# vovach777/llcomp

Measured on AMD Instinct MI355X. Metric: encode+decode MPix/s on 4K RGB8, bit-exact, higher is better.
Workload: dtype int32

## Files before the change

### llcomp_amd/csrc/dec_rows_asm.hpp

```cpp
#pragma once
#include <cstdint>

namespace llcomp_mi {

#define LD_E0L "v32"
#define LD_E0H "v33"
#define LD_E0 "v[32:33]"
#define LD_E5L "v34"
#define LD_E5H "v35"
#define LD_E5 "v[34:35]"
#define LD_E6L "v36"
#define LD_E6H "v37"
#define LD_E6 "v[36:37]"
#define LD_E7L "v38"
#define LD_E7H "v39"
#define LD_E7 "v[38:39]"
#define LD_E1L "v40"
#define LD_E1H "v41"
#define LD_E1 "v[40:41]"
#define LD_E2L "v42"
#define LD_E2H "v43"
#define LD_E2 "v[42:43]"
#define LD_E3L "v44"
#define LD_E3H "v45"
#define LD_E3 "v[44:45]"
#define LD_E4L "v48"
#define LD_E4H "v49"
#define LD_E4 "v[48:49]"
#define LD_PROD "v50"
#define LD_R1 "v51"
#define LD_DIFF "v52"
#define LD_OFF "v52"
#define LD_EX "v32"
#define LD_W "v33"
#define LD_RUN "v40"
#define LD_NX "v41"
#define LD_T "v42"
#define LD_SX "s[56:57]"
#define LD_SA "s[58:59]"
#define LD_SW "s[60:61]"
#define LD_SP "s[62:63]"
#define LD_S5 "s[64:65]"
#define LD_SU "s[66:67]"
#define LD_SD "s[68:69]"
#define LD_S1L "s[68:69]"
#define LD_SM "s[70:71]"
#define LD_S1 "s70"
#define LD_S2 "s71"

#define LD_SPLIT(EL)                                                                                                       \
    "v_mul_u32_u24_sdwa " LD_PROD ", " EL ", %[range] dst_sel:DWORD dst_unused:UNUSED_PAD src0_sel:BYTE_1 src1_sel:DWORD\n\t" \
    "v_lshrrev_b32_e32 " LD_R1 ", 8, " LD_PROD "\n\t"                                                                      \
    "v_sub_u32_e32 %[range], %[range], " LD_R1 "\n\t"
#define LD_SPLIT_IN(EL)                                                                                                       \
    "v_mul_u32_u24_sdwa " LD_PROD ", " EL ", %[range_in] dst_sel:DWORD dst_unused:UNUSED_PAD src0_sel:BYTE_1 src1_sel:DWORD\n\t" \
    "v_lshrrev_b32_e32 " LD_R1 ", 8, " LD_PROD "\n\t"                                                                      \
    "v_sub_u32_e32 %[range], %[range_in], " LD_R1 "\n\t"
#define LD_REFILL(N)                                         \
    "v_cmp_gt_u32_e32 vcc, %[c100], %[range]\n\t"            \
    "s_and_saveexec_b64 " LD_SW ", vcc\n\t"                  \
    "s_cbranch_execz .Lrf" N "_%=\n\t"                       \
    "v_lshlrev_b32_e32 %[range], 8, %[range]\n\t"            \
    "v_perm_b32 %[low], %[low], %[w32], %[sel]\n\t"          \
    "v_lshrrev_b32_e32 %[w32], 8, %[w32]\n"                   \
    ".Lrf" N "_%=:\n\t"                                      \
    "s_mov_b64 exec, " LD_SW "\n\t"
#define LD_REFILL_R1(N)                                           \
    "v_cmp_gt_u32_e32 vcc, %[c100], " LD_R1 "\n\t"                \
    "s_and_saveexec_b64 " LD_SW ", vcc\n\t"                       \
    "s_cbranch_execz .Lrf" N "_%=\n\t"                            \
    "v_and_b32_e32 %[range], 0xffffff00, " LD_PROD "\n\t"         \
    "v_perm_b32 %[low], %[low], %[w32], %[sel]\n\t"               \
    "v_lshrrev_b32_e32 %[w32], 8, %[w32]\n"                        \
    ".Lrf" N "_%=:\n\t"                                           \
    "s_mov_b64 exec, " LD_SW "\n\t"
#define LD_UNARY(EL, EH, OFS, N, SAVE)                                      \
    LD_SPLIT(EL)                                                            \
    "v_sub_co_u32_e32 %[low], vcc, %[low], %[range]\n\t"                    \
    "ds_write_b16_d16_hi %[bank], " EL " offset:" OFS "\n\t"                \
    "s_andn2_b64 exec, exec, vcc\n\t"                                       \
    SAVE                                                                    \
    "s_cbranch_execz .Lx_done_%=\n\t"                                       \
    "ds_write_b16_d16_hi %[bank], " EH " offset:" OFS "\n\t"                \
    "v_add_u32_e32 " LD_EX ", 1, " LD_EX "\n\t"                                     \
    "v_mov_b32_e32 %[range], " LD_R1 "\n\t"                                 \
    LD_REFILL_R1(N)
#define LD_FETCH_REST                                         \
    "v_lshrrev_b32_e32 " LD_E1L ", 16, %[w0]\n\t"             \
    "v_and_b32_e32 " LD_E2L ", 0xffff, %[w1]\n\t"             \
    "v_lshrrev_b32_e32 " LD_E3L ", 16, %[w1]\n\t"             \
    "v_and_b32_e32 " LD_E4L ", 0xffff, %[w2]\n\t"             \
    "ds_read_b64 " LD_E1 ", " LD_E1L "\n\t"                   \
    "ds_read_b64 " LD_E2 ", " LD_E2L "\n\t"                   \
    "ds_read_b64 " LD_E3 ", " LD_E3L "\n\t"                   \
    "ds_read_b64 " LD_E4 ", " LD_E4L "\n\t"                   \
    "v_lshrrev_b32_e32 " LD_E5L ", 16, %[w2]\n\t"             \
    "v_and_b32_e32 " LD_E6L ", 0xffff, %[w3]\n\t"             \
    "v_lshrrev_b32_e32 " LD_E7L ", 16, %[w3]\n\t"             \
    "ds_read_b64 " LD_E5 ", " LD_E5L "\n\t"                   \
    "ds_read_b64 " LD_E6 ", " LD_E6L "\n\t"                   \
    "ds_read_b64 " LD_E7 ", " LD_E7L "\n\t"

__device__ __forceinline__ void dec_rows_sample_asm(uint32_t low_in, uint32_t range_in, unsigned long long win_in, uint32_t& low,
                                                    uint32_t& range, unsigned long long& win, uint32_t w0, uint32_t w1, uint32_t w2,
                                                    uint32_t w3, uint32_t bank, uint32_t& hot, uint32_t& value, uint32_t& w32) {
    asm volatile(
        "s_mov_b64 " LD_SX ", exec\n\t"
        "v_and_b32_e32 %[w32], 0xffffff, %[winl_in]\n\t"
        "v_or_b32_e32 %[w32], 0x1000000, %[w32]\n\t"
        "v_and_b32_e32 " LD_OFF ", 0xffff, %[w0]\n\t"
        "ds_read_b64 " LD_E0 ", " LD_OFF "\n\t"
        "v_mov_b32_e32 %[value], 0\n\t"
        "s_cmp_lg_u32 %[hot], 0\n\t"
        "s_cbranch_scc0 .Lcold_%=\n\t"
        LD_FETCH_REST
        "s_waitcnt lgkmcnt(7)\n\t"
        "s_branch .Lzero_%=\n"
        ".Lcold_%=:\n\t"
        "s_waitcnt lgkmcnt(0)\n"
        ".Lzero_%=:\n\t"
        LD_SPLIT_IN(LD_E0L)
        "v_sub_co_u32_e32 %[low], vcc, %[low_in], %[range]\n\t"
        "ds_write_b16_d16_hi %[bank], " LD_E0L "\n\t"
        "s_and_b64 " LD_SA ", exec, vcc\n\t"
        "v_cndmask_b32_e32 %[low], %[low], %[low_in], vcc\n\t"
        "s_andn2_b64 exec, exec, vcc\n\t"
        "s_cbranch_execz .Lz1_%=\n\t"
        "v_mov_b32_e32 %[range], " LD_R1 "\n\t"
        "ds_write_b16_d16_hi %[bank], " LD_E0H "\n"
        ".Lz1_%=:\n\t"
        "s_mov_b64 exec, " LD_SX "\n\t"
        LD_REFILL("0")
        "s_and_b64 exec, " LD_SA ", " LD_SA "\n\t"
        "s_cbranch_execz .Ldone_%=\n\t"
        "s_cmp_lg_u32 %[hot], 0\n\t"
        "s_cbranch_scc1 .Lhave_%=\n\t"
        LD_FETCH_REST
        ".Lhave_%=:\n\t"
        "v_mov_b32_e32 " LD_EX ", 0\n\t"
        "v_mov_b32_e32 " LD_W ", 1\n\t"
        "s_waitcnt lgkmcnt(0)\n\t"
        "s_mov_b64 " LD_SM ", 0\n\t"
        LD_UNARY(LD_E1L, LD_E1H, "2", "1", "s_mov_b64 " LD_S1L ", exec\n\t")
        LD_UNARY(LD_E2L, LD_E2H, "256", "2", "s_mov_b64 " LD_SM ", exec\n\t")
        LD_UNARY(LD_E3L, LD_E3H, "258", "3", "")
        "s_mov_b64 " LD_SU ", exec\n\t"
        ".p2align 6\n"
        ".Lu_%=:\n\t"
        "s_waitcnt lgkmcnt(0)\n\t"
        LD_SPLIT(LD_E4L)
        "v_sub_co_u32_e32 %[low], vcc, %[low], %[range]\n\t"
        "s_andn2_b64 exec, exec, vcc\n\t"
        "s_cbranch_execz .Lu_done_%=\n\t"
        "v_lshrrev_b32_e32 " LD_OFF ", 16, " LD_E4H "\n\t"
        "ds_read_b64 " LD_E4 ", " LD_OFF "\n\t"
        "v_add_u32_e32 " LD_EX ", 1, " LD_EX "\n\t"
        "v_mov_b32_e32 %[range], " LD_R1 "\n\t"
        LD_REFILL_R1("4")
        "s_branch .Lu_%=\n"
        ".Lu_done_%=:\n\t"
        "s_mov_b64 exec, " LD_SU "\n\t"
        "ds_write_b16_d16_hi %[bank], " LD_E4L " offset:512\n"
        ".Lx_done_%=:\n\t"
        "s_mov_b64 exec, " LD_SA "\n\t"
        "v_add_u32_e32 %[low], %[low], %[range]\n\t"
        LD_REFILL("5")
        "v_cmp_lt_u32_e32 vcc, 31, " LD_EX "\n\t"
        "s_cbranch_vccz .Lexok_%=\n\t"
        "s_and_saveexec_b64 " LD_SP ", vcc\n\t"
        "v_mov_b32_e32 %[w32], 0\n\t"
        "s_andn2_b64 exec, " LD_SP ", exec\n\t"
        "s_cbranch_execz .Ldone_%=\n"
        ".Lexok_%=:\n\t"
        "s_mov_b64 " LD_S5 ", exec\n\t"
        "s_and_b64 exec, exec, " LD_S1L "\n\t"
        "s_cbranch_execz .Lvalue_%=\n\t"
        "s_mov_b64 " LD_SU ", exec\n\t"
        LD_SPLIT(LD_E5L)
        "v_sub_co_u32_e32 " LD_DIFF ", vcc, %[low], %[range]\n\t"
        "ds_write_b16_d16_hi %[bank], " LD_E5L " offset:514\n\t"
        "s_andn2_b64 " LD_SP ", exec, vcc\n\t"
        "v_addc_co_u32_e32 " LD_W ", vcc, " LD_W ", " LD_W ", vcc\n\t"
        "v_mov_b32_e32 " LD_RUN ", 0\n\t"
        "s_and_b64 exec, " LD_SP ", " LD_SP "\n\t"
        "s_cbranch_execz .Lp5_%=\n\t"
        "v_mov_b32_e32 %[low], " LD_DIFF "\n\t"
        "v_mov_b32_e32 %[range], " LD_R1 "\n\t"
        "ds_write_b16_d16_hi %[bank], " LD_E5H " offset:514\n"
        ".Lp5_%=:\n\t"
        "s_mov_b64 exec, " LD_SU "\n\t"
        LD_REFILL("6")
        "v_add_u32_e32 " LD_T ", -1, " LD_EX "\n\t"
        "s_and_b64 exec, exec, " LD_SM "\n\t"
        "s_cbranch_execz .Lm_skip_%=\n\t"
        "s_mov_b64 " LD_SP ", exec\n\t"
        "v_add_u32_e32 " LD_NX ", -2, " LD_EX "\n\t"
        "v_lshrrev_b32_e32 " LD_RUN ", " LD_NX ", %[sentv]\n\t"
        ".p2align 6\n"
        ".Lm_%=:\n\t"
        "s_waitcnt lgkmcnt(0)\n\t"
        LD_SPLIT(LD_E6L)
        "v_sub_co_u32_e32 " LD_DIFF ", vcc, %[low], %[range]\n\t"
        "s_nop 1\n\t"
        "v_cndmask_b32_e32 %[range], " LD_R1 ", %[range], vcc\n\t"
        "v_cndmask_b32_e32 %[low], " LD_DIFF ", %[low], vcc\n\t"
        "v_cndmask_b32_e32 " LD_NX ", " LD_E6H ", " LD_E6L ", vcc\n\t"
        "v_addc_co_u32_e32 " LD_RUN ", vcc, " LD_RUN ", " LD_RUN ", vcc\n\t"
        "s_mov_b64 " LD_SD ", vcc\n\t"
        "v_lshrrev_b32_e32 " LD_OFF ", 16, " LD_NX "\n\t"
        "ds_read_b64 " LD_E6 ", " LD_OFF "\n\t"
        "v_cmp_gt_u32_e32 vcc, %[c100], %[range]\n\t"
        "s_and_saveexec_b64 " LD_SW ", vcc\n\t"
        "s_cbranch_execz .Lmr_%=\n\t"
        "v_lshlrev_b32_e32 %[range], 8, %[range]\n\t"
        "v_perm_b32 %[low], %[low], %[w32], %[sel]\n\t"
        "v_lshrrev_b32_e32 %[w32], 8, %[w32]\n"
        ".Lmr_%=:\n\t"
        "s_andn2_b64 exec, " LD_SW ", " LD_SD "\n\t"
        "s_cbranch_execnz .Lm_%=\n\t"
        "s_mov_b64 exec, " LD_SP "\n\t"
        "ds_write_b16_d16_hi %[bank], " LD_NX " offset:768\n"
        ".Lm_skip_%=:\n\t"
        "s_mov_b64 exec, " LD_SU "\n\t"
        "v_lshlrev_b32_e32 " LD_W ", " LD_T ", " LD_W "\n\t"
        "v_or_b32_e32 " LD_W ", " LD_W ", " LD_RUN "\n"
        ".Lvalue_%=:\n\t"
        "s_mov_b64 exec, " LD_S5 "\n\t"
        "v_lshlrev_b32_e64 " LD_T ", " LD_EX ", 1\n\t"
        "v_add_u32_e32 " LD_T ", -1, " LD_T "\n\t"
        "v_xor_b32_e32 %[value], " LD_W ", " LD_T "\n\t"
        LD_SPLIT(LD_E7L)
        "v_sub_co_u32_e32 " LD_DIFF ", vcc, %[low], %[range]\n\t"
        "ds_write_b16_d16_hi %[bank], " LD_E7L " offset:770\n\t"
        "s_andn2_b64 exec, exec, vcc\n\t"
        "s_cbranch_execz .Lp7_%=\n\t"
        "v_mov_b32_e32 %[low], " LD_DIFF "\n\t"
        "v_mov_b32_e32 %[range], " LD_R1 "\n\t"
        "ds_write_b16_d16_hi %[bank], " LD_E7H " offset:770\n\t"
        "v_sub_u32_e32 %[value], 0, %[value]\n"
        ".Lp7_%=:\n\t"
        "s_mov_b64 exec, " LD_S5 "\n\t"
        LD_REFILL("7")
        ".Ldone_%=:\n\t"
        "s_mov_b64 exec, " LD_SX "\n\t"
        "v_ffbh_u32_e32 " LD_DIFF ", %[w32]\n\t"
        "v_add_u32_e32 " LD_DIFF ", -7, " LD_DIFF "\n\t"
        "v_lshrrev_b64 %[win], " LD_DIFF ", %[win_in]\n\t"
        "s_bcnt1_i32_b64 " LD_S1 ", " LD_SA "\n\t"
        "s_bcnt1_i32_b64 " LD_S2 ", " LD_SX "\n\t"
        "s_lshl_b32 " LD_S1 ", " LD_S1 ", 1\n\t"
        "s_cmp_ge_u32 " LD_S1 ", " LD_S2 "\n\t"
        "s_cselect_b32 %[hot], 1, 0\n\t"
        "s_mov_b64 exec, " LD_SX "\n\t"
        : [low] "=&v"(low), [range] "=&v"(range), [win] "=&v"(win), [hot] "+s"(hot), [value] "=&v"(value), [w32] "=&v"(w32)
        : [low_in] "v"(low_in), [range_in] "v"(range_in), [win_in] "v"(win_in), [winl_in] "v"(uint32_t(win_in)), [w0] "v"(w0), [w1] "v"(w1), [w2] "v"(w2), [w3] "v"(w3), [bank] "v"(bank), [c100] "s"(0x100u), [sel] "s"(0x06050400u),
          [sentv] "v"(0x80000000u)
        : "vcc", "scc", "memory", "v32", "v33", "v34", "v35", "v36", "v37", "v38", "v39", "v40", "v41", "v42", "v43", "v44", "v45",
          "v48", "v49", "v50", "v51", "v52", "s56", "s57", "s58", "s59", "s60", "s61", "s62", "s63", "s64", "s65", "s66",
          "s67", "s68", "s69", "s70", "s71");
}

}
```

### llcomp_amd/csrc/slice_kernels.hip

```cpp
#include <algorithm>
#include <type_traits>

#include "device_common.hpp"
#include "kernels.hpp"

#ifndef LLMI_ASM_ENC
#define LLMI_ASM_ENC 1
#endif
#if LLMI_ASM_ENC
#include "enc_rows_asm.hpp"
#endif
#ifndef LLMI_ASM_DEC
#define LLMI_ASM_DEC 1
#endif
#if LLMI_ASM_DEC
#include "dec_rows_asm.hpp"
#endif

namespace llcomp_mi {

namespace {

#ifdef LLMI_CLOCK_PROBE
constexpr uint32_t kProbeSlots = 1u << 15;
// ... 869 lines not shown
    bool ok = true;
    if (dec_once<1, CHECKED, INLDS>(d, bank, E)) {
        ex = 1;
        if (dec_once<2, CHECKED, INLDS>(d, bank, E)) {
            ex = 2;
            if (dec_once<3, CHECKED, INLDS>(d, bank, E)) {
                entry_t cur = E.e4;
                int n = 0;
                for (;;) {
                    if (CHECKED && d.win <= 1) dec_append_drained(d);
                    const uint32_t r1 = __umul24(d.range, prob_of(cur)) >> 8;
                    d.range -= r1;
                    ++n;
                    asm volatile("" : "+v"(n));
                    uint32_t diff;
                    if (__builtin_usub_overflow(d.low, d.range, &diff)) break;
                    d.low = diff;
                    d.range = r1;
                    if (CHECKED && n > 29) break;
                    cur = entry_at(tab, uint32_t(cur >> 32));
                    dec_refill(d);
                }
                dec_refill(d);
                ex = 2 + n;
                if (ex > 31) ok = false;
                const uint32_t nx = uint32_t(cur);
                dec_put_state<4, INLDS>(bank, nx);
            }
        }
    }
    if (!ok) return false;
    uint32_t w = 1;
    const uint32_t ones = (1u << ex) - 1;
    if (ex > 0) {
        w += w + uint32_t(!dec_once<5, CHECKED, INLDS>(d, bank, E));
        if (ex > 1) {
            entry_t cur = E.e6;
            uint32_t nx;
            uint32_t limit = ones + 1;
            asm volatile("" : "+v"(limit));
            do {
                nx = dec_step_acc<CHECKED>(d, prob_of(cur), cur, w);
                cur = entry_at(tab, nx);
            } while (w < limit);
            dec_put_state<6, INLDS>(bank, nx);
        }
    }
    uint32_t v = w ^ ones;
    if (dec_once<7, CHECKED, INLDS>(d, bank, E)) v = 0u - v;
    out = v;
    return true;
}

template <bool INLDS>
__device__ __forceinline__ bool dec_sample(RangeDec& d, Bank& bank, const entry_t* tab, uint32_t& hot, bool replay_always,
                                           uint32_t& v) {
#if LLMI_ASM_DEC
    if constexpr (INLDS) {
        uint32_t low, range, left;
        unsigned long long win;
        dec_rows_sample_asm(d.low, d.range, d.win, low, range, win, bank.w[0], bank.w[1], bank.w[2], bank.w[3], lds_address(bank.lds), hot, v,
                            left);
        if (__builtin_expect(left == 0 || replay_always, 0)) {
            ++d.replays;
            reinterpret_cast<uint32_t*>(bank.lds)[0] = bank.w[0];
            reinterpret_cast<uint32_t*>(bank.lds)[64] = bank.w[1];
            reinterpret_cast<uint32_t*>(bank.lds)[128] = bank.w[2];
            reinterpret_cast<uint32_t*>(bank.lds)[192] = bank.w[3];
            asm("v_mov_b32_e32 %0, %3\n\tv_mov_b32_e32 %1, %4\n\tv_mov_b64_e32 %2, %5"
                : "+v"(low), "+v"(range), "+v"(win)
                : "v"(d.low), "v"(d.range), "v"(d.win));
            d.low = low;
            d.range = range;
            d.win = win;
            return dec_residual<false, true, true>(d, bank, tab, v);
        }
        d.low = low;
        d.range = range;
        d.win = win;
        return true;
    } else
#endif
    {
        const uint32_t s_low = d.low, s_range = d.range, s_b0 = bank.w[0], s_b1 = bank.w[1], s_b2 = bank.w[2], s_b3 = bank.w[3];
        const unsigned long long s_win = d.win;
        bool ok = hot ? dec_residual<true, false, INLDS>(d, bank, tab, v) : dec_residual<false, false, INLDS>(d, bank, tab, v);
        hot = 2 * __popcll(__ballot(v != 0)) >= __popcll(__ballot(true));
        if (__builtin_expect(!ok || d.win == 0 || replay_always, 0)) {
            ++d.replays;
            d.low = s_low; d.range = s_range; d.win = s_win;
            bank.w[0] = s_b0; bank.w[1] = s_b1;
            if constexpr (INLDS) {
                bank.w[2] = s_b2; bank.w[3] = s_b3;
                reinterpret_cast<uint32_t*>(bank.lds)[0] = s_b0;
                reinterpret_cast<uint32_t*>(bank.lds)[64] = s_b1;
                reinterpret_cast<uint32_t*>(bank.lds)[128] = s_b2;
                reinterpret_cast<uint32_t*>(bank.lds)[192] = s_b3;
            }
            ok = dec_residual<false, true, INLDS>(d, bank, tab, v);
        }
        return ok;
    }
}

constexpr uint32_t bank_cache_lds_bytes(int log2_entries) { return log2_entries ? (64u * 9u) << log2_entries : 0u; }
template <int NCH, bool ROWS, bool LDSTAB = false, int CACHE = 0, bool SMALL = false>
__global__ __launch_bounds__(64, ROWS && NCH == 1 ? 8 : 1) void k_decode_slices(const Geometry g, const uint32_t lpw_and_flags,
                                                      const uint8_t* __restrict__ units,
                                                      const uint32_t* __restrict__ slice_len,
                                                      uint64_t* __restrict__ states, int16_t* __restrict__ rec,
                                                      uint32_t* status, const uint64_t gpat,
                                                      unsigned long long* __restrict__ counters) {
    __shared__ entry_t tab[128];
    __shared__ uint32_t rowbank[ROWS ? kWideBankWords : 1];
    __shared__ int8_t quant_lut[ROWS ? 1 : 512];
    if constexpr (!ROWS) {
        for (uint32_t i = threadIdx.x; i < 256; i += blockDim.x) {
            quant_lut[i] = int8_t(quant11(int(i) - 128));
            quant_lut[256 + i] = int8_t(quant5(int(i) - 128));
        }
    }
    static_assert(CACHE == 0 || (!ROWS && !LDSTAB && NCH != 0), "the bank cache belongs to the 2-D kernels with tables in HBM");
    static_assert(!SMALL || ROWS, "the model is a template flag of the 1-row-slice kernels only");
    static_assert(CACHE == 0 || ((kContexts - 1) >> CACHE) < 0xFF, "bank cache: a context's tag would alias the empty marker");
    __shared__ uint32_t wave_sums[CACHE != 0 ? 2 : 1];
    clear_lds_states<LDSTAB>();
    if constexpr (CACHE != 0) {
        uint32_t* tg = reinterpret_cast<uint32_t*>(dyn_lds + (512u << CACHE));
        for (uint32_t i = threadIdx.x; i < (16u << CACHE); i += blockDim.x) tg[i] = 0xFFFFFFFFu;
        if (threadIdx.x < 2) wave_sums[threadIdx.x] = 0;
    }
    load_table(tab);
    const uint32_t lpw = lpw_and_flags & 0xFF;
    const bool replay_always = (lpw_and_flags >> 8) & 1;
    [[maybe_unused]] const bool small_model = (g.flags & kGeoSmallModel) != 0;
    const uint32_t id = blockIdx.x * lpw + threadIdx.x;
    if (threadIdx.x >= lpw || id >= g.n_slices) return;
    const SliceRect r = slice_rect(g, id);
    RangeDec d;
    const uint32_t len = min(slice_len[id], g.slice_cap - 16);
    const uint32_t grp = __builtin_amdgcn_readfirstlane(id >> g.lane_shift);
    const uint32_t lane_in_group = id & ((1u << g.lane_shift) - 1);
    dec_open(d, reinterpret_cast<const uint32_t*>(units) + ((size_t(grp) * (g.slice_cap >> 2)) << g.lane_shift), lane_in_group,
             g.lane_shift, len);

    int16_t* p0 = rec + lane_order_index(g, id, 0);
    const ptrdiff_t GW = ptrdiff_t(1) << g.lane_shift;
    int16_t* const gbase = rec + ((size_t(grp) * g.slice_samples) << g.lane_shift);
    uint32_t hot = 0;
    LLMI_PROBE_START();

    if constexpr (ROWS) {
        for (uint32_t k = 0; k < 12; ++k) rowbank[k * 64 + threadIdx.x] = lds_address(tab) * 0x00010001u;
        int l[NCH], L[NCH];
#pragma unroll
        for (int k = 0; k < NCH; ++k) l[k] = L[k] = 128;
        int held_val = 0;
        uint32_t store_ofs = lane_in_group * 2, step_ofs = 2u << g.lane_shift;
        asm volatile("" : "+v"(step_ofs));
        uint8_t* const bank0 = reinterpret_cast<uint8_t*>(rowbank) + threadIdx.x * 4;
        bool bad = false;
        auto pixel = [&](auto model, auto start) {
            constexpr int MODEL = decltype(model)::value;
            constexpr bool START = decltype(start)::value;
#pragma unroll
            for (int k = 0; k < NCH; ++k) {
                if (window_low(d)) dec_append(d);
                if (!(START && k == 0)) {
                    asm volatile("global_store_short %0, %1, %2" : : "v"(store_ofs), "v"(held_val), "s"(gbase) : "memory");
                    store_ofs += step_ofs;
                }
                const int lv = l[k];
                uint32_t sg = 0, bofs = 0;
                if constexpr (MODEL != kModelSmall) {
                    const int dq = L[k] - lv;
                    sg = uint32_t(dq >> 31);
                    asm volatile("" : "+v"(sg));
                    const uint32_t aq = (uint32_t(dq) ^ sg) - sg;
                    uint32_t o1 = ((aq + 0x7FFFFFFFu) >> 21) & 0x400u, o2 = ((aq + 0x7FFFFFFCu) >> 21) & 0x400u;
                    asm volatile("" : "+v"(o1), "+v"(o2));
                    bofs = o1 + o2;
                }
                uint32_t* bp = reinterpret_cast<uint32_t*>(bank0 + bofs);
                Bank bank{{bp[0], bp[64], bp[128], bp[192]}, reinterpret_cast<uint8_t*>(bp)};
                uint32_t v = 0;
                if (!dec_sample<true>(d, bank, tab, hot, replay_always, v)) bad = true;
                if constexpr (MODEL != kModelSmall) v = (v ^ sg) - sg;
                const int val = int(int16_t(uint32_t(lv) + v));
                held_val = val;
                L[k] = START ? val : lv;
                l[k] = val;
            }
        };
        const uint32_t sw0 = __builtin_amdgcn_readfirstlane(r.sw);
        const uint32_t n_bulk = __builtin_amdgcn_ballot_w64(r.sw != sw0) == 0 ? sw0 : 0;
        uint32_t x = 1;
        pixel(no_model, std::true_type{});
        constexpr std::integral_constant<int, SMALL ? kModelSmall : kModelLarge> model{};
        if constexpr (NCH == 1) {
            for (; x + 1 < n_bulk; x += 2) {
                pixel(model, std::false_type{});
                pixel(model, std::false_type{});
            }
        } else {
            for (; x < n_bulk; ++x) pixel(model, std::false_type{});
        }
        for (; x < r.sw; ++x) pixel(model, std::false_type{});
        if (bad) atomicOr(status, kStBadExponent);
        asm volatile("global_store_short %0, %1, %2" : : "v"(store_ofs), "v"(held_val), "s"(gbase) : "memory");
        publish_count(counters, kCtrDecReplays, d.replays);
    } else {
        uint64_t* banks;
        uint32_t bsh;
        if constexpr (LDSTAB) {
            banks = reinterpret_cast<uint64_t*>(dyn_lds);
            bsh = 0;
        } else {
            banks = states + ((size_t(id >> g.lane_shift) * kContexts) << g.lane_shift) + (id & ((1u << g.lane_shift) - 1));
            bsh = g.lane_shift;
        }
        if constexpr (NCH == 0) {
            const uint32_t nch = g.nch;
            const ptrdiff_t px_step = ptrdiff_t(nch) * GW, up = ptrdiff_t(r.sw) * px_step;
            for (uint32_t y = 0; y < r.sh; ++y) {
                for (uint32_t x = 0; x < r.sw; ++x) {
                    for (uint32_t k = 0; k < nch; ++k) {
                        int16_t* q = p0 + ptrdiff_t(y) * up + ptrdiff_t(x) * px_step + ptrdiff_t(k) * GW;
                        if (window_low(d)) dec_append(d);
                        const Hood n = apply_borders(x > 0 ? q[-px_step] : 0, x > 1 ? q[-2 * px_step] : 0, y > 0 ? q[-up] : 0,
                                                     (y > 0 && x > 0) ? q[-up - px_step] : 0, (y > 0 && x + 1 < r.sw) ? q[-up + px_step] : 0,
                                                     y > 1 ? q[-2 * up] : 0, x, y, r.sw);
                        int ctx = context_hash(n, small_model);
                        const bool neg = ctx < 0;
                        if (neg) ctx = -ctx;
                        const uint64_t b64 = bank_fresh<LDSTAB>(banks[size_t(ctx) << bsh], gpat);
                        Bank bank{{uint32_t(b64), uint32_t(b64 >> 32)}, nullptr};
                        uint32_t v;
                        if (!dec_sample<false>(d, bank, tab, hot, replay_always, v)) {
                            atomicOr(status, kStBadExponent);
                            return;
                        }
                                banks[size_t(ctx) << bsh] = bank_tagged<LDSTAB>(uint64_t(bank.w[0]) | (uint64_t(bank.w[1]) << 32), gpat);
                        if (neg) v = 0u - v;
                        *q = int16_t(uint32_t(predict(n)) + v);
                    }
                }
            }
            publish_count(counters, kCtrDecReplays, d.replays);
        } else {
        const ptrdiff_t up = ptrdiff_t(r.sw) * NCH * GW;
        uint32_t held_ctx = ~0u;
        uint64_t held_bank = 0;
        [[maybe_unused]] uint64_t wb_bank = 0;
        [[maybe_unused]] uint64_t* wb_ptr = nullptr;
        [[maybe_unused]] bool use_cache = CACHE != 0;
        [[maybe_unused]] uint32_t my_miss = 0, my_lookups = 0, my_wb = 0, miss_mark = 0, look_mark = 0;
        LLMI_PARTS_DECL();
        LLMI_PARTS_START();
        for (uint32_t y = 0; y < r.sh; ++y) {
            if constexpr (CACHE != 0) {
// ... 273 lines not shown
```

Before: 30460.

## Pack decoder low and byte window into a 64-bit register pair with alternating sets

Rewrites the row-decoder inline assembly so the range-coder low value and the pending refill bytes sit in one 64-bit register pair. A refill then becomes a single 64-bit shift in place of a perm plus a shift. The unary-run loop is unrolled by two, with range and R1 swapping roles so the register move per step disappears. Consecutive samples alternate between two fixed register pairs (v0:1 / v2:3), which lets the compiler overlap them and avoid copies. The cost is hard-pinned physical registers and more complex asm that must stay bit-exact.

```diff
diff --git a/llcomp_amd/csrc/dec_rows_asm.hpp b/llcomp_amd/csrc/dec_rows_asm.hpp
--- a/llcomp_amd/csrc/dec_rows_asm.hpp
+++ b/llcomp_amd/csrc/dec_rows_asm.hpp
@@ -41,6 +41,7 @@
 #define LD_SW "s[60:61]"
 #define LD_SP "s[62:63]"
 #define LD_S5 "s[64:65]"
+#define LD_SB "s[64:65]"
 #define LD_SU "s[66:67]"
 #define LD_SD "s[68:69]"
 #define LD_S1L "s[68:69]"
@@ -56,35 +57,37 @@
     "v_mul_u32_u24_sdwa " LD_PROD ", " EL ", %[range_in] dst_sel:DWORD dst_unused:UNUSED_PAD src0_sel:BYTE_1 src1_sel:DWORD\n\t" \
     "v_lshrrev_b32_e32 " LD_R1 ", 8, " LD_PROD "\n\t"                                                                      \
     "v_sub_u32_e32 %[range], %[range_in], " LD_R1 "\n\t"
+#define LD_SPLIT_TO(EL, RD, WR)                                                                                       \
+    "v_mul_u32_u24_sdwa " LD_PROD ", " EL ", " RD " dst_sel:DWORD dst_unused:UNUSED_PAD src0_sel:BYTE_1 src1_sel:DWORD\n\t" \
+    "v_lshrrev_b32_e32 " WR ", 8, " LD_PROD "\n\t"                                                                     \
+    "v_sub_u32_e32 " RD ", " RD ", " WR "\n\t"
+#define LD_TAKE "v_lshlrev_b64 " LD_PAIR ", 8, " LD_PAIR "\n"
 #define LD_REFILL(N)                                         \
     "v_cmp_gt_u32_e32 vcc, %[c100], %[range]\n\t"            \
     "s_and_saveexec_b64 " LD_SW ", vcc\n\t"                  \
     "s_cbranch_execz .Lrf" N "_%=\n\t"                       \
     "v_lshlrev_b32_e32 %[range], 8, %[range]\n\t"            \
-    "v_perm_b32 %[low], %[low], %[w32], %[sel]\n\t"          \
-    "v_lshrrev_b32_e32 %[w32], 8, %[w32]\n"                   \
+    LD_TAKE                                                  \
     ".Lrf" N "_%=:\n\t"                                      \
     "s_mov_b64 exec, " LD_SW "\n\t"
-#define LD_REFILL_R1(N)                                           \
-    "v_cmp_gt_u32_e32 vcc, %[c100], " LD_R1 "\n\t"                \
+#define LD_REFILL_R1(WR, N)                                       \
+    "v_cmp_gt_u32_e32 vcc, %[c100], " WR "\n\t"                   \
     "s_and_saveexec_b64 " LD_SW ", vcc\n\t"                       \
     "s_cbranch_execz .Lrf" N "_%=\n\t"                            \
-    "v_and_b32_e32 %[range], 0xffffff00, " LD_PROD "\n\t"         \
-    "v_perm_b32 %[low], %[low], %[w32], %[sel]\n\t"               \
-    "v_lshrrev_b32_e32 %[w32], 8, %[w32]\n"                        \
+    "v_and_b32_e32 " WR ", 0xffffff00, " LD_PROD "\n\t"           \
+    LD_TAKE                                                       \
     ".Lrf" N "_%=:\n\t"                                           \
     "s_mov_b64 exec, " LD_SW "\n\t"
-#define LD_UNARY(EL, EH, OFS, N, SAVE)                                      \
-    LD_SPLIT(EL)                                                            \
-    "v_sub_co_u32_e32 %[low], vcc, %[low], %[range]\n\t"                    \
+#define LD_UNARY(EL, EH, OFS, N, SAVE, RD, WR)                              \
+    LD_SPLIT_TO(EL, RD, WR)                                                 \
+    "v_sub_co_u32_e32 " LD_LOW ", vcc, " LD_LOW ", " RD "\n\t"              \
     "ds_write_b16_d16_hi %[bank], " EL " offset:" OFS "\n\t"                \
     "s_andn2_b64 exec, exec, vcc\n\t"                                       \
     SAVE                                                                    \
     "s_cbranch_execz .Lx_done_%=\n\t"                                       \
     "ds_write_b16_d16_hi %[bank], " EH " offset:" OFS "\n\t"                \
-    "v_add_u32_e32 " LD_EX ", 1, " LD_EX "\n\t"                                     \
-    "v_mov_b32_e32 %[range], " LD_R1 "\n\t"                                 \
-    LD_REFILL_R1(N)
+    "v_add_u32_e32 " LD_EX ", 1, " LD_EX "\n\t"                             \
+    LD_REFILL_R1(WR, N)
 #define LD_FETCH_REST                                         \
     "v_lshrrev_b32_e32 " LD_E1L ", 16, %[w0]\n\t"             \
     "v_and_b32_e32 " LD_E2L ", 0xffff, %[w1]\n\t"             \
@@ -101,163 +104,233 @@
     "ds_read_b64 " LD_E6 ", " LD_E6L "\n\t"                   \
     "ds_read_b64 " LD_E7 ", " LD_E7L "\n\t"
 
-__device__ __forceinline__ void dec_rows_sample_asm(uint32_t low_in, uint32_t range_in, unsigned long long win_in, uint32_t& low,
-                                                    uint32_t& range, unsigned long long& win, uint32_t w0, uint32_t w1, uint32_t w2,
-                                                    uint32_t w3, uint32_t bank, uint32_t& hot, uint32_t& value, uint32_t& w32) {
-    asm volatile(
-        "s_mov_b64 " LD_SX ", exec\n\t"
-        "v_and_b32_e32 %[w32], 0xffffff, %[winl_in]\n\t"
-        "v_or_b32_e32 %[w32], 0x1000000, %[w32]\n\t"
-        "v_and_b32_e32 " LD_OFF ", 0xffff, %[w0]\n\t"
-        "ds_read_b64 " LD_E0 ", " LD_OFF "\n\t"
-        "v_mov_b32_e32 %[value], 0\n\t"
-        "s_cmp_lg_u32 %[hot], 0\n\t"
-        "s_cbranch_scc0 .Lcold_%=\n\t"
-        LD_FETCH_REST
-        "s_waitcnt lgkmcnt(7)\n\t"
-        "s_branch .Lzero_%=\n"
-        ".Lcold_%=:\n\t"
-        "s_waitcnt lgkmcnt(0)\n"
-        ".Lzero_%=:\n\t"
-        LD_SPLIT_IN(LD_E0L)
-        "v_sub_co_u32_e32 %[low], vcc, %[low_in], %[range]\n\t"
-        "ds_write_b16_d16_hi %[bank], " LD_E0L "\n\t"
-        "s_and_b64 " LD_SA ", exec, vcc\n\t"
-        "v_cndmask_b32_e32 %[low], %[low], %[low_in], vcc\n\t"
-        "s_andn2_b64 exec, exec, vcc\n\t"
-        "s_cbranch_execz .Lz1_%=\n\t"
-        "v_mov_b32_e32 %[range], " LD_R1 "\n\t"
-        "ds_write_b16_d16_hi %[bank], " LD_E0H "\n"
-        ".Lz1_%=:\n\t"
+#define LD_HEAD_COPY "v_perm_b32 " LD_CPY ", %[winl_in], %[winl_in], %[sel]\n\t"
+#define LD_SEL 0x0001020Du
+#define LD_TAIL_BITS "v_ffbl_b32_e32 " LD_DIFF ", " LD_CPY "\n\t"
+#define LD_URUN                                                      \
+    ".Lu_%=:\n\t"                                                    \
+    "s_waitcnt lgkmcnt(0)\n\t"                                       \
+    LD_SPLIT_TO(LD_E4L, LD_R1, "%[range]")                           \
+    "v_sub_co_u32_e32 " LD_LOW ", vcc, " LD_LOW ", " LD_R1 "\n\t"    \
+    "s_and_b64 " LD_SP ", exec, vcc\n\t"                             \
+    "s_andn2_b64 exec, exec, vcc\n\t"                                \
+    "s_or_b64 " LD_SB ", " LD_SB ", " LD_SP "\n\t"                   \
+    "s_cbranch_execz .Lu_done_%=\n\t"                                \
+    "v_lshrrev_b32_e32 " LD_OFF ", 16, " LD_E4H "\n\t"               \
+    "ds_read_b64 " LD_E4 ", " LD_OFF "\n\t"                          \
+    "v_add_u32_e32 " LD_EX ", 1, " LD_EX "\n\t"                      \
+    LD_REFILL_R1("%[range]", "4")                                    \
+    "s_waitcnt lgkmcnt(0)\n\t"                                       \
+    LD_SPLIT_TO(LD_E4L, "%[range]", LD_R1)                           \
+    "v_sub_co_u32_e32 " LD_LOW ", vcc, " LD_LOW ", %[range]\n\t"     \
+    "s_andn2_b64 exec, exec, vcc\n\t"                                \
+    "s_cbranch_execz .Lu_done_%=\n\t"                                \
+    "v_lshrrev_b32_e32 " LD_OFF ", 16, " LD_E4H "\n\t"               \
+    "ds_read_b64 " LD_E4 ", " LD_OFF "\n\t"                          \
+    "v_add_u32_e32 " LD_EX ", 1, " LD_EX "\n\t"                      \
+    LD_REFILL_R1(LD_R1, "4b")                                        \
+    "s_branch .Lu_%=\n"
+#define LD_UNARY_INIT "s_mov_b64 " LD_SB ", 0\n\t"
+#define LD_SAVE2 "s_mov_b64 " LD_SM ", exec\n\ts_andn2_b64 " LD_SB ", " LD_S1L ", exec\n\t"
+#define LD_COLLECT                           \
+    "s_mov_b64 exec, " LD_SB "\n\t"          \
+    "v_mov_b32_e32 %[range], " LD_R1 "\n\t"
+
+#define LD_TEXT                                                                                                                    \
+        "s_mov_b64 " LD_SX ", exec\n\t"                                                                                            \
+        LD_HEAD_COPY                                                                                                               \
+        "v_and_b32_e32 " LD_OFF ", 0xffff, %[w0]\n\t"                                                                              \
+        "ds_read_b64 " LD_E0 ", " LD_OFF "\n\t"                                                                                    \
+        "v_mov_b32_e32 %[value], 0\n\t"                                                                                            \
+        "s_cmp_lg_u32 %[hot], 0\n\t"                                                                                               \
+        "s_cbranch_scc0 .Lcold_%=\n\t"                                                                                             \
+        LD_FETCH_REST                                                                                                              \
+        "s_waitcnt lgkmcnt(7)\n\t"                                                                                                 \
+        "s_branch .Lzero_%=\n"                                                                                                     \
+        ".Lcold_%=:\n\t"                                                                                                           \
+        "s_waitcnt lgkmcnt(0)\n"                                                                                                   \
+                                       \
+        ".Lzero_%=:\n\t"                                                                                                           \
+           \
+                                          \
+        LD_SPLIT_IN(LD_E0L)                                                                                                        \
+        "v_sub_co_u32_e32 " LD_LOW ", vcc, %[low_in], %[range]\n\t"                                                                \
+        "ds_write_b16_d16_hi %[bank], " LD_E0L "\n\t"                                                                              \
+        "s_and_b64 " LD_SA ", exec, vcc\n\t"                                                                                       \
+        "v_cndmask_b32_e32 " LD_LOW ", " LD_LOW ", %[low_in], vcc\n\t"                                                             \
+        "s_andn2_b64 exec, exec, vcc\n\t"                                                                                          \
+        "s_cbranch_execz .Lz1_%=\n\t"                                                                                              \
+        "v_mov_b32_e32 %[range], " LD_R1 "\n\t"                                                                                    \
+        "ds_write_b16_d16_hi %[bank], " LD_E0H "\n"                                                                                \
+        ".Lz1_%=:\n\t"                                                                                                             \
+        "s_mov_b64 exec, " LD_SX "\n\t"                                                                                            \
+        LD_REFILL("0")                                                                                                             \
+        "s_and_b64 exec, " LD_SA ", " LD_SA "\n\t"                                                                                 \
+        "s_cbranch_execz .Ldone_%=\n\t"                                                                                            \
+        "s_cmp_lg_u32 %[hot], 0\n\t"                                                                                               \
+        "s_cbranch_scc1 .Lhave_%=\n\t"                                                                                             \
+        LD_FETCH_REST                                                                                                              \
+        ".Lhave_%=:\n\t"                                                                                                           \
+        "v_mov_b32_e32 " LD_EX ", 0\n\t"                                                                                           \
+        "v_mov_b32_e32 " LD_W ", 1\n\t"                                                                                            \
+        "s_waitcnt lgkmcnt(0)\n\t"                                                                                                 \
+                    \
+           \
+                                                       \
+        "s_mov_b64 " LD_SM ", 0\n\t"                                                                                               \
+        LD_UNARY_INIT                                                                                                              \
+        LD_UNARY(LD_E1L, LD_E1H, "2", "1", "s_mov_b64 " LD_S1L ", exec\n\t", "%[range]", LD_R1)                                   \
+        LD_UNARY(LD_E2L, LD_E2H, "256", "2", LD_SAVE2, LD_R1, "%[range]")                                                          \
+        LD_UNARY(LD_E3L, LD_E3H, "258", "3", "", "%[range]", LD_R1)                                                                \
+        "s_mov_b64 " LD_SU ", exec\n\t"                                                                                            \
+        ".p2align 6\n"                                                                                                             \
+        LD_URUN                                                                                                                    \
+        ".Lu_done_%=:\n\t"                                                                                                         \
+        "s_mov_b64 exec, " LD_SU "\n\t"                                                                                            \
+        "ds_write_b16_d16_hi %[bank], " LD_E4L " offset:512\n"                             \
+        ".Lx_done_%=:\n\t"                                                                                                         \
+        LD_COLLECT                                                                                                                 \
+        "s_mov_b64 exec, " LD_SA "\n\t"                                                                                            \
+        "v_add_u32_e32 " LD_LOW ", " LD_LOW ", %[range]\n\t"     \
+        LD_REFILL("5")                                                                   \
+                                 \
+        "v_cmp_lt_u32_e32 vcc, 31, " LD_EX "\n\t"                                                                                  \
+        "s_cbranch_vccz .Lexok_%=\n\t"                                                                                             \
+        "s_and_saveexec_b64 " LD_SP ", vcc\n\t"                                                                                    \
+        "v_mov_b32_e32 " LD_CPY ", 0\n\t"        \
+        "s_andn2_b64 exec, " LD_SP ", exec\n\t"                                                                                    \
+        "s_cbranch_execz .Ldone_%=\n"                                                                                              \
+        ".Lexok_%=:\n\t"                                                                                                           \
+        "s_mov_b64 " LD_S5 ", exec\n\t"                             \
+                                    \
+        "s_and_b64 exec, exec, " LD_S1L "\n\t"                                                                  \
+        "s_cbranch_execz .Lvalue_%=\n\t"                                                                                           \
+        "s_mov_b64 " LD_SU ", exec\n\t"                                                                                            \
+        LD_SPLIT(LD_E5L)                                                                                                           \
+        "v_sub_co_u32_e32 " LD_DIFF ", vcc, " LD_LOW ", %[range]\n\t"                                                              \
+        "ds_write_b16_d16_hi %[bank], " LD_E5L " offset:514\n\t"                                                                   \
+        "s_andn2_b64 " LD_SP ", exec, vcc\n\t"                                                    \
+        "v_addc_co_u32_e32 " LD_W ", vcc, " LD_W ", " LD_W ", vcc\n\t"                                        \
+        "v_mov_b32_e32 " LD_RUN ", 0\n\t"                                                                                          \
+        "s_and_b64 exec, " LD_SP ", " LD_SP "\n\t"                                                                                 \
+        "s_cbranch_execz .Lp5_%=\n\t"                                                                                              \
+        "v_mov_b32_e32 " LD_LOW ", " LD_DIFF "\n\t"                                                                                \
+        "v_mov_b32_e32 %[range], " LD_R1 "\n\t"                                                                                    \
+        "ds_write_b16_d16_hi %[bank], " LD_E5H " offset:514\n"                                                                     \
+        ".Lp5_%=:\n\t"                                                                                                             \
+        "s_mov_b64 exec, " LD_SU "\n\t"                                                                                            \
+        LD_REFILL("6")                                                                                                             \
+         \
+        "v_add_u32_e32 " LD_T ", -1, " LD_EX "\n\t"                                                      \
+        "s_and_b64 exec, exec, " LD_SM "\n\t"                                                                   \
+        "s_cbranch_execz .Lm_skip_%=\n\t"                                                                                          \
+        "s_mov_b64 " LD_SP ", exec\n\t"                                                                                            \
+        "v_add_u32_e32 " LD_NX ", -2, " LD_EX "\n\t"                                                                               \
+        "v_lshrrev_b32_e32 " LD_RUN ", " LD_NX ", %[sentv]\n\t"                                         \
+        ".p2align 6\n"                                                                                                             \
+        ".Lm_%=:\n\t"                                                                                                              \
+        "s_waitcnt lgkmcnt(0)\n\t"                                                                                                 \
+        LD_SPLIT(LD_E6L)                                                                                                           \
+        "v_sub_co_u32_e32 " LD_DIFF ", vcc, " LD_LOW ", %[range]\n\t"                                                              \
+        "s_nop 1\n\t"                                            \
+        "v_cndmask_b32_e32 %[range], " LD_R1 ", %[range], vcc\n\t"                                                                 \
+        "v_cndmask_b32_e32 " LD_LOW ", " LD_DIFF ", " LD_LOW ", vcc\n\t"                                                           \
+        "v_cndmask_b32_e32 " LD_NX ", " LD_E6H ", " LD_E6L ", vcc\n\t"                                                             \
+                                                            \
+        "v_addc_co_u32_e32 " LD_RUN ", vcc, " LD_RUN ", " LD_RUN ", vcc\n\t"                                                       \
+        "s_mov_b64 " LD_SD ", vcc\n\t"                                                                                             \
+        "v_lshrrev_b32_e32 " LD_OFF ", 16, " LD_NX "\n\t"                                                                          \
+        "ds_read_b64 " LD_E6 ", " LD_OFF "\n\t"                                                                                    \
+        "v_cmp_gt_u32_e32 vcc, %[c100], %[range]\n\t"                                                                              \
+        "s_and_saveexec_b64 " LD_SW ", vcc\n\t"                                                                                    \
+        "s_cbranch_execz .Lmr_%=\n\t"                                                                                              \
+        "v_lshlrev_b32_e32 %[range], 8, %[range]\n\t"                                                                              \
+        LD_TAKE                                                                                                                    \
+        ".Lmr_%=:\n\t"                                                                                                             \
+        "s_andn2_b64 exec, " LD_SW ", " LD_SD "\n\t"                           \
+        "s_cbranch_execnz .Lm_%=\n\t"                                                                                              \
+        "s_mov_b64 exec, " LD_SP "\n\t"                                                                                            \
+        "ds_write_b16_d16_hi %[bank], " LD_NX " offset:768\n"                       \
+        ".Lm_skip_%=:\n\t"                                                                                                         \
+        "s_mov_b64 exec, " LD_SU "\n\t"                                                                                            \
+        "v_lshlrev_b32_e32 " LD_W ", " LD_T ", " LD_W "\n\t"   \
+        "v_or_b32_e32 " LD_W ", " LD_W ", " LD_RUN "\n"                                                                            \
+                                 \
+        ".Lvalue_%=:\n\t"                                                                                                          \
+        "s_mov_b64 exec, " LD_S5 "\n\t"                                                                                            \
+        "v_lshlrev_b32_e64 " LD_T ", " LD_EX ", 1\n\t"                                                                             \
+        "v_add_u32_e32 " LD_T ", -1, " LD_T "\n\t"                                                                                 \
+        "v_xor_b32_e32 %[value], " LD_W ", " LD_T "\n\t"                                                                           \
+                                                                                      \
+        LD_SPLIT(LD_E7L)                                                                                                           \
+        "v_sub_co_u32_e32 " LD_DIFF ", vcc, " LD_LOW ", %[range]\n\t"                                                              \
+        "ds_write_b16_d16_hi %[bank], " LD_E7L " offset:770\n\t"                                                                   \
+        "s_andn2_b64 exec, exec, vcc\n\t"                                                                                          \
+        "s_cbranch_execz .Lp7_%=\n\t"                                                                                              \
+        "v_mov_b32_e32 " LD_LOW ", " LD_DIFF "\n\t"                                                                                \
+        "v_mov_b32_e32 %[range], " LD_R1 "\n\t"                                                                                    \
+        "ds_write_b16_d16_hi %[bank], " LD_E7H " offset:770\n\t"                                                                   \
+        "v_sub_u32_e32 %[value], 0, %[value]\n"                                                                                    \
+        ".Lp7_%=:\n\t"                                                                                                             \
+        "s_mov_b64 exec, " LD_S5 "\n\t"                                                                                            \
+        LD_REFILL("7")                                                                                                             \
+        ".Ldone_%=:\n\t"                                                                                                           \
+        "s_mov_b64 exec, " LD_SX "\n\t"                                                                                            \
+        LD_TAIL_BITS                                                                                                               \
+        "v_lshrrev_b64 %[win], " LD_DIFF ", %[win_in]\n\t"              \
+        "s_bcnt1_i32_b64 " LD_S1 ", " LD_SA "\n\t"                                                                                 \
+        "s_bcnt1_i32_b64 " LD_S2 ", " LD_SX "\n\t"                                                                                 \
+        "s_lshl_b32 " LD_S1 ", " LD_S1 ", 1\n\t"                                                                                   \
+        "s_cmp_ge_u32 " LD_S1 ", " LD_S2 "\n\t"                                                                                    \
+        "s_cselect_b32 %[hot], 1, 0\n\t"                                                                                           \
         "s_mov_b64 exec, " LD_SX "\n\t"
-        LD_REFILL("0")
-        "s_and_b64 exec, " LD_SA ", " LD_SA "\n\t"
-        "s_cbranch_execz .Ldone_%=\n\t"
-        "s_cmp_lg_u32 %[hot], 0\n\t"
-        "s_cbranch_scc1 .Lhave_%=\n\t"
-        LD_FETCH_REST
-        ".Lhave_%=:\n\t"
-        "v_mov_b32_e32 " LD_EX ", 0\n\t"
-        "v_mov_b32_e32 " LD_W ", 1\n\t"
-        "s_waitcnt lgkmcnt(0)\n\t"
-        "s_mov_b64 " LD_SM ", 0\n\t"
-        LD_UNARY(LD_E1L, LD_E1H, "2", "1", "s_mov_b64 " LD_S1L ", exec\n\t")
-        LD_UNARY(LD_E2L, LD_E2H, "256", "2", "s_mov_b64 " LD_SM ", exec\n\t")
-        LD_UNARY(LD_E3L, LD_E3H, "258", "3", "")
-        "s_mov_b64 " LD_SU ", exec\n\t"
-        ".p2align 6\n"
-        ".Lu_%=:\n\t"
-        "s_waitcnt lgkmcnt(0)\n\t"
-        LD_SPLIT(LD_E4L)
-        "v_sub_co_u32_e32 %[low], vcc, %[low], %[range]\n\t"
-        "s_andn2_b64 exec, exec, vcc\n\t"
-        "s_cbranch_execz .Lu_done_%=\n\t"
-        "v_lshrrev_b32_e32 " LD_OFF ", 16, " LD_E4H "\n\t"
-        "ds_read_b64 " LD_E4 ", " LD_OFF "\n\t"
-        "v_add_u32_e32 " LD_EX ", 1, " LD_EX "\n\t"
-        "v_mov_b32_e32 %[range], " LD_R1 "\n\t"
-        LD_REFILL_R1("4")
-        "s_branch .Lu_%=\n"
-        ".Lu_done_%=:\n\t"
-        "s_mov_b64 exec, " LD_SU "\n\t"
-        "ds_write_b16_d16_hi %[bank], " LD_E4L " offset:512\n"
-        ".Lx_done_%=:\n\t"
-        "s_mov_b64 exec, " LD_SA "\n\t"
-        "v_add_u32_e32 %[low], %[low], %[range]\n\t"
-        LD_REFILL("5")
-        "v_cmp_lt_u32_e32 vcc, 31, " LD_EX "\n\t"
-        "s_cbranch_vccz .Lexok_%=\n\t"
-        "s_and_saveexec_b64 " LD_SP ", vcc\n\t"
-        "v_mov_b32_e32 %[w32], 0\n\t"
-        "s_andn2_b64 exec, " LD_SP ", exec\n\t"
-        "s_cbranch_execz .Ldone_%=\n"
-        ".Lexok_%=:\n\t"
-        "s_mov_b64 " LD_S5 ", exec\n\t"
-        "s_and_b64 exec, exec, " LD_S1L "\n\t"
-        "s_cbranch_execz .Lvalue_%=\n\t"
-        "s_mov_b64 " LD_SU ", exec\n\t"
-        LD_SPLIT(LD_E5L)
-        "v_sub_co_u32_e32 " LD_DIFF ", vcc, %[low], %[range]\n\t"
-        "ds_write_b16_d16_hi %[bank], " LD_E5L " offset:514\n\t"
-        "s_andn2_b64 " LD_SP ", exec, vcc\n\t"
-        "v_addc_co_u32_e32 " LD_W ", vcc, " LD_W ", " LD_W ", vcc\n\t"
-        "v_mov_b32_e32 " LD_RUN ", 0\n\t"
-        "s_and_b64 exec, " LD_SP ", " LD_SP "\n\t"
-        "s_cbranch_execz .Lp5_%=\n\t"
-        "v_mov_b32_e32 %[low], " LD_DIFF "\n\t"
-        "v_mov_b32_e32 %[range], " LD_R1 "\n\t"
-        "ds_write_b16_d16_hi %[bank], " LD_E5H " offset:514\n"
-        ".Lp5_%=:\n\t"
-        "s_mov_b64 exec, " LD_SU "\n\t"
-        LD_REFILL("6")
-        "v_add_u32_e32 " LD_T ", -1, " LD_EX "\n\t"
-        "s_and_b64 exec, exec, " LD_SM "\n\t"
-        "s_cbranch_execz .Lm_skip_%=\n\t"
-        "s_mov_b64 " LD_SP ", exec\n\t"
-        "v_add_u32_e32 " LD_NX ", -2, " LD_EX "\n\t"
-        "v_lshrrev_b32_e32 " LD_RUN ", " LD_NX ", %[sentv]\n\t"
-        ".p2align 6\n"
-        ".Lm_%=:\n\t"
-        "s_waitcnt lgkmcnt(0)\n\t"
-        LD_SPLIT(LD_E6L)
-        "v_sub_co_u32_e32 " LD_DIFF ", vcc, %[low], %[range]\n\t"
-        "s_nop 1\n\t"
-        "v_cndmask_b32_e32 %[range], " LD_R1 ", %[range], vcc\n\t"
-        "v_cndmask_b32_e32 %[low], " LD_DIFF ", %[low], vcc\n\t"
-        "v_cndmask_b32_e32 " LD_NX ", " LD_E6H ", " LD_E6L ", vcc\n\t"
-        "v_addc_co_u32_e32 " LD_RUN ", vcc, " LD_RUN ", " LD_RUN ", vcc\n\t"
-        "s_mov_b64 " LD_SD ", vcc\n\t"
-        "v_lshrrev_b32_e32 " LD_OFF ", 16, " LD_NX "\n\t"
-        "ds_read_b64 " LD_E6 ", " LD_OFF "\n\t"
-        "v_cmp_gt_u32_e32 vcc, %[c100], %[range]\n\t"
-        "s_and_saveexec_b64 " LD_SW ", vcc\n\t"
-        "s_cbranch_execz .Lmr_%=\n\t"
-        "v_lshlrev_b32_e32 %[range], 8, %[range]\n\t"
-        "v_perm_b32 %[low], %[low], %[w32], %[sel]\n\t"
-        "v_lshrrev_b32_e32 %[w32], 8, %[w32]\n"
-        ".Lmr_%=:\n\t"
-        "s_andn2_b64 exec, " LD_SW ", " LD_SD "\n\t"
-        "s_cbranch_execnz .Lm_%=\n\t"
-        "s_mov_b64 exec, " LD_SP "\n\t"
-        "ds_write_b16_d16_hi %[bank], " LD_NX " offset:768\n"
-        ".Lm_skip_%=:\n\t"
-        "s_mov_b64 exec, " LD_SU "\n\t"
-        "v_lshlrev_b32_e32 " LD_W ", " LD_T ", " LD_W "\n\t"
-        "v_or_b32_e32 " LD_W ", " LD_W ", " LD_RUN "\n"
-        ".Lvalue_%=:\n\t"
-        "s_mov_b64 exec, " LD_S5 "\n\t"
-        "v_lshlrev_b32_e64 " LD_T ", " LD_EX ", 1\n\t"
-        "v_add_u32_e32 " LD_T ", -1, " LD_T "\n\t"
-        "v_xor_b32_e32 %[value], " LD_W ", " LD_T "\n\t"
-        LD_SPLIT(LD_E7L)
-        "v_sub_co_u32_e32 " LD_DIFF ", vcc, %[low], %[range]\n\t"
-        "ds_write_b16_d16_hi %[bank], " LD_E7L " offset:770\n\t"
-        "s_andn2_b64 exec, exec, vcc\n\t"
-        "s_cbranch_execz .Lp7_%=\n\t"
-        "v_mov_b32_e32 %[low], " LD_DIFF "\n\t"
-        "v_mov_b32_e32 %[range], " LD_R1 "\n\t"
-        "ds_write_b16_d16_hi %[bank], " LD_E7H " offset:770\n\t"
-        "v_sub_u32_e32 %[value], 0, %[value]\n"
-        ".Lp7_%=:\n\t"
-        "s_mov_b64 exec, " LD_S5 "\n\t"
-        LD_REFILL("7")
-        ".Ldone_%=:\n\t"
-        "s_mov_b64 exec, " LD_SX "\n\t"
-        "v_ffbh_u32_e32 " LD_DIFF ", %[w32]\n\t"
-        "v_add_u32_e32 " LD_DIFF ", -7, " LD_DIFF "\n\t"
-        "v_lshrrev_b64 %[win], " LD_DIFF ", %[win_in]\n\t"
-        "s_bcnt1_i32_b64 " LD_S1 ", " LD_SA "\n\t"
-        "s_bcnt1_i32_b64 " LD_S2 ", " LD_SX "\n\t"
-        "s_lshl_b32 " LD_S1 ", " LD_S1 ", 1\n\t"
-        "s_cmp_ge_u32 " LD_S1 ", " LD_S2 "\n\t"
-        "s_cselect_b32 %[hot], 1, 0\n\t"
-        "s_mov_b64 exec, " LD_SX "\n\t"
-        : [low] "=&v"(low), [range] "=&v"(range), [win] "=&v"(win), [hot] "+s"(hot), [value] "=&v"(value), [w32] "=&v"(w32)
-        : [low_in] "v"(low_in), [range_in] "v"(range_in), [win_in] "v"(win_in), [winl_in] "v"(uint32_t(win_in)), [w0] "v"(w0), [w1] "v"(w1), [w2] "v"(w2), [w3] "v"(w3), [bank] "v"(bank), [c100] "s"(0x100u), [sel] "s"(0x06050400u),
-          [sentv] "v"(0x80000000u)
-        : "vcc", "scc", "memory", "v32", "v33", "v34", "v35", "v36", "v37", "v38", "v39", "v40", "v41", "v42", "v43", "v44", "v45",
-          "v48", "v49", "v50", "v51", "v52", "s56", "s57", "s58", "s59", "s60", "s61", "s62", "s63", "s64", "s65", "s66",
-          "s67", "s68", "s69", "s70", "s71");
+#define LD_INPUTS                                                                                                                   \
+    [low_in] "v"(low_in), [range_in] "v"(range_in), [win_in] "v"(win_in), [winl_in] "v"(uint32_t(win_in)), [w0] "v"(w0), [w1] "v"(w1), \
+        [w2] "v"(w2), [w3] "v"(w3), [bank] "v"(bank), [c100] "s"(0x100u), [sel] "s"(LD_SEL), [sentv] "v"(0x80000000u)
+#define LD_CLOBBERS                                                                                                                 \
+    "vcc", "scc", "memory", "v32", "v33", "v34", "v35", "v36", "v37", "v38", "v39", "v40", "v41", "v42", "v43", "v44", "v45", "v48", \
+        "v49", "v50", "v51", "v52", "s56", "s57", "s58", "s59", "s60", "s61", "s62", "s63", "s64", "s65", "s66", "s67", "s68", "s69", \
+        "s70", "s71"
+
+#define LD_BLOCK(PAIR)                                                                                                        \
+    asm volatile(LD_TEXT : [lc] "=&{" PAIR "}"(low_copy), [range] "=&v"(range), [win] "=&v"(win), [hot] "+s"(hot), [value] "=&v"(value) \
+                 : LD_INPUTS                                                                                                  \
+                 : LD_CLOBBERS)
+#define LD_REPLAY_COPY(PAIR)                                                                  \
+    asm("v_mov_b32_e32 " LD_LOW ", %3\n\tv_mov_b32_e32 %1, %4\n\tv_mov_b64_e32 %2, %5"        \
+        : "+{" PAIR "}"(low_copy), "+v"(range), "+v"(win)                                     \
+        : "v"(low_in), "v"(range_in), "v"(win_in))
+template <int SET>
+__device__ __forceinline__ void dec_rows_sample_asm(uint32_t low_in, uint32_t range_in, unsigned long long win_in,
+                                                    unsigned long long& low_copy, uint32_t& range, unsigned long long& win, uint32_t w0,
+                                                    uint32_t w1, uint32_t w2, uint32_t w3, uint32_t bank, uint32_t& hot, uint32_t& value) {
+    if constexpr (SET == 0) {
+#define LD_PAIR "v[0:1]"
+#define LD_CPY "v0"
+#define LD_LOW "v1"
+        LD_BLOCK("v[0:1]");
+    } else {
+#undef LD_PAIR
+#undef LD_CPY
+#undef LD_LOW
+#define LD_PAIR "v[2:3]"
+#define LD_CPY "v2"
+#define LD_LOW "v3"
+        LD_BLOCK("v[2:3]");
+    }
 }
-
+template <int SET>
+__device__ __forceinline__ void dec_rows_replay_inputs(uint32_t low_in, uint32_t range_in, unsigned long long win_in,
+                                                       unsigned long long& low_copy, uint32_t& range, unsigned long long& win) {
+    if constexpr (SET == 0) {
+#undef LD_LOW
+#define LD_LOW "v1"
+        LD_REPLAY_COPY("v[0:1]");
+    } else {
+#undef LD_LOW
+#define LD_LOW "v3"
+        LD_REPLAY_COPY("v[2:3]");
+    }
 }
+
+}
diff --git a/llcomp_amd/csrc/slice_kernels.hip b/llcomp_amd/csrc/slice_kernels.hip
--- a/llcomp_amd/csrc/slice_kernels.hip
+++ b/llcomp_amd/csrc/slice_kernels.hip
@@ -945,30 +945,28 @@
     return true;
 }
 
-template <bool INLDS>
+template <bool INLDS, int SET = 0>
 __device__ __forceinline__ bool dec_sample(RangeDec& d, Bank& bank, const entry_t* tab, uint32_t& hot, bool replay_always,
                                            uint32_t& v) {
 #if LLMI_ASM_DEC
     if constexpr (INLDS) {
-        uint32_t low, range, left;
-        unsigned long long win;
-        dec_rows_sample_asm(d.low, d.range, d.win, low, range, win, bank.w[0], bank.w[1], bank.w[2], bank.w[3], lds_address(bank.lds), hot, v,
-                            left);
-        if (__builtin_expect(left == 0 || replay_always, 0)) {
+        uint32_t range;
+        unsigned long long low_left, win;
+        dec_rows_sample_asm<SET>(d.low, d.range, d.win, low_left, range, win, bank.w[0], bank.w[1], bank.w[2], bank.w[3], lds_address(bank.lds),
+                                 hot, v);
+        if (__builtin_expect(uint32_t(low_left) == 0 || replay_always, 0)) {
             ++d.replays;
             reinterpret_cast<uint32_t*>(bank.lds)[0] = bank.w[0];
             reinterpret_cast<uint32_t*>(bank.lds)[64] = bank.w[1];
             reinterpret_cast<uint32_t*>(bank.lds)[128] = bank.w[2];
             reinterpret_cast<uint32_t*>(bank.lds)[192] = bank.w[3];
-            asm("v_mov_b32_e32 %0, %3\n\tv_mov_b32_e32 %1, %4\n\tv_mov_b64_e32 %2, %5"
-                : "+v"(low), "+v"(range), "+v"(win)
-                : "v"(d.low), "v"(d.range), "v"(d.win));
-            d.low = low;
+            dec_rows_replay_inputs<SET>(d.low, d.range, d.win, low_left, range, win);
+            d.low = uint32_t(low_left >> 32);
             d.range = range;
             d.win = win;
             return dec_residual<false, true, true>(d, bank, tab, v);
         }
-        d.low = low;
+        d.low = uint32_t(low_left >> 32);
         d.range = range;
         d.win = win;
         return true;
@@ -1053,9 +1051,10 @@
         asm volatile("" : "+v"(step_ofs));
         uint8_t* const bank0 = reinterpret_cast<uint8_t*>(rowbank) + threadIdx.x * 4;
         bool bad = false;
-        auto pixel = [&](auto model, auto start) {
+        auto pixel = [&](auto model, auto start, auto set) {
             constexpr int MODEL = decltype(model)::value;
             constexpr bool START = decltype(start)::value;
+            constexpr int SET = decltype(set)::value;
 #pragma unroll
             for (int k = 0; k < NCH; ++k) {
                 if (window_low(d)) dec_append(d);
@@ -1077,7 +1076,9 @@
                 uint32_t* bp = reinterpret_cast<uint32_t*>(bank0 + bofs);
                 Bank bank{{bp[0], bp[64], bp[128], bp[192]}, reinterpret_cast<uint8_t*>(bp)};
                 uint32_t v = 0;
-                if (!dec_sample<true>(d, bank, tab, hot, replay_always, v)) bad = true;
+                const bool ok = ((SET + k) & 1) ? dec_sample<true, 1>(d, bank, tab, hot, replay_always, v)
+                                                : dec_sample<true, 0>(d, bank, tab, hot, replay_always, v);
+                if (!ok) bad = true;
                 if constexpr (MODEL != kModelSmall) v = (v ^ sg) - sg;
                 const int val = int(int16_t(uint32_t(lv) + v));
                 held_val = val;
@@ -1088,17 +1089,19 @@
         const uint32_t sw0 = __builtin_amdgcn_readfirstlane(r.sw);
         const uint32_t n_bulk = __builtin_amdgcn_ballot_w64(r.sw != sw0) == 0 ? sw0 : 0;
         uint32_t x = 1;
-        pixel(no_model, std::true_type{});
+        constexpr std::integral_constant<int, 0> set0{};
+        constexpr std::integral_constant<int, 1> set1{};
+        pixel(no_model, std::true_type{}, set0);
         constexpr std::integral_constant<int, SMALL ? kModelSmall : kModelLarge> model{};
         if constexpr (NCH == 1) {
             for (; x + 1 < n_bulk; x += 2) {
-                pixel(model, std::false_type{});
-                pixel(model, std::false_type{});
+                pixel(model, std::false_type{}, set1);
+                pixel(model, std::false_type{}, set0);
             }
         } else {
-            for (; x < n_bulk; ++x) pixel(model, std::false_type{});
-        }
-        for (; x < r.sw; ++x) pixel(model, std::false_type{});
+            for (; x < n_bulk; ++x) pixel(model, std::false_type{}, set0);
+        }
+        for (; x < r.sw; ++x) pixel(model, std::false_type{}, set1);
         if (bad) atomicOr(status, kStBadExponent);
         asm volatile("global_store_short %0, %1, %2" : : "v"(store_ofs), "v"(held_val), "s"(gbase) : "memory");
         publish_count(counters, kCtrDecReplays, d.replays);
```

After: 30830, median of 6. +1.2%, better.
